# gstoica27/ReLUQP-py

Hardware: AMD Instinct MI355X
Metric: QP solves/sec (batch=4096 random dense QPs n=100 m=300) (higher is better)
Workload: dtype f32; 1 GPU; batch=4096/GPU random dense QPs n=100 m=300 (n_eq=25), feasible rand_qp seeds 0.., eps_abs=0.001, cold start, reference defaults; 4 distinct batches in rotation, every solve without dispatch history (= first solve of a fresh handle); global_batch=4096, parallelism=batch-split x1, no collectives, kernel=resident2, tile=same, low_memory=False, fresh_batches=4, dispatch_history=False, rho_window=5

## Files before the change

reluqp-py_amd/csrc/rqp_resident2.hip:

```cpp
#include <cstdio>
#include <cstdlib>
#include <type_traits>
#include <vector>

#include "rqp_common.h"

typedef float f2 __attribute__((ext_vector_type(2)));
typedef _Float16 h2 __attribute__((ext_vector_type(2)));

__device__ __forceinline__ float fma_mix_lo(h2 k, float v, float acc) {
    asm("v_fma_mix_f32 %0, %1, %2, %0 op_sel_hi:[1,0,0]" : "+v"(acc) : "v"(k), "v"(v));
    return acc;
}
__device__ __forceinline__ float fma_mix_hi(h2 k, float v, float acc) {
    asm("v_fma_mix_f32 %0, %1, %2, %0 op_sel:[1,0,0] op_sel_hi:[1,0,0]" : "+v"(acc) : "v"(k), "v"(v));
    return acc;
}
template <int CTRL>
__device__ __forceinline__ float dpp2(float v) {
    return __builtin_bit_cast(float, __builtin_amdgcn_update_dpp(0, __builtin_bit_cast(int, v), CTRL, 0xF, 0xF, true));
}
__device__ __forceinline__ float swsum32(float a, float b) {
    asm volatile("s_nop 1\n\tv_permlane32_swap_b32 %0, %1" : "+v"(a), "+v"(b));
    return a + b;
}
__device__ __forceinline__ float swsum16(float a, float b) {
    asm volatile("s_nop 1\n\tv_permlane16_swap_b32 %0, %1" : "+v"(a), "+v"(b));
    return a + b;
}
__device__ __forceinline__ float swmax32(float a, float b) {
    asm volatile("s_nop 1\n\tv_permlane32_swap_b32 %0, %1" : "+v"(a), "+v"(b));
    return fmaxf(a, b);
}
__device__ __forceinline__ float swmax16(float a, float b) {
    asm volatile("s_nop 1\n\tv_permlane16_swap_b32 %0, %1" : "+v"(a), "+v"(b));
    return fmaxf(a, b);
}
__device__ __forceinline__ float wave_max(float v) {
    v = fmaxf(v, dpp2<0xB1>(v));
    v = fmaxf(v, dpp2<0x4E>(v));
    v = fmaxf(v, dpp2<0x141>(v));
    v = fmaxf(v, dpp2<0x128>(v));
    float a = v, b = v;
    asm volatile("s_nop 1\n\tv_permlane16_swap_b32 %0, %1" : "+v"(a), "+v"(b));
    v = fmaxf(a, b);
    a = v; b = v;
    asm volatile("s_nop 1\n\tv_permlane32_swap_b32 %0, %1" : "+v"(a), "+v"(b));
    return fmaxf(a, b);
}
__device__ __forceinline__ unsigned wave_or(unsigned v) {
    v |= (unsigned)__builtin_amdgcn_update_dpp(0, (int)v, 0xB1, 0xF, 0xF, true);
    v |= (unsigned)__builtin_amdgcn_update_dpp(0, (int)v, 0x4E, 0xF, 0xF, true);
    v |= (unsigned)__builtin_amdgcn_update_dpp(0, (int)v, 0x141, 0xF, 0xF, true);
    v |= (unsigned)__builtin_amdgcn_update_dpp(0, (int)v, 0x128, 0xF, 0xF, true);
    unsigned a = v, b = v;
    asm volatile("s_nop 1\n\tv_permlane16_swap_b32 %0, %1" : "+v"(a), "+v"(b));
    v = a | b;
    a = v; b = v;
    asm volatile("s_nop 1\n\tv_permlane32_swap_b32 %0, %1" : "+v"(a), "+v"(b));
    return a | b;
}
template <typename T>
__device__ __forceinline__ T tmax2(T a, T b) {
    return (a != a) ? a : ((b != b) ? b : (a > b ? a : b));
}

template <int RB_, int CQ_, int KR_, int KC_>
struct Res2Cfg {
    static constexpr int RB = RB_, CQ = CQ_, KR = KR_, KC = KC_;
    static constexpr int NT = 256, NW = 4, NQ = 2, PL = 32;
    static constexpr int RP = RB / 2, KP = KR / 2;
    static constexpr int CW = NQ * CQ;
    static constexpr int N = NW * CW;
    static constexpr int M = PL * RB;
    static constexpr int SW = 8 * KR + 4;
    static constexpr int ND = NW * SW;
    static constexpr int AE2 = RP * CQ;
    static constexpr int KE2 = KP * KC;
    static constexpr int HR = 4, HP = HR / 2;
    static constexpr int HE2 = HP * CQ;
    static constexpr int HU = HE2 / 2;
    static constexpr int H1 = (CQ + 1) / 2, H2 = (H1 + 1) / 2;
    static constexpr int MATREGS = 2 * (RP * CQ + KP * KC);
    static constexpr int WAVES_PER_SIMD = (MATREGS > 100) ? 2 : ((MATREGS > 30) ? 3 : 4);
    static_assert(RB % 2 == 0 && KR % 2 == 0 && HP == 2 && HU == CQ && PL * HR >= N, "row pairs");
    static_assert(8 * KR >= CW && 8 * KC >= N && M <= 2 * NT && KC == CQ && NQ == 2, "tile shape");
    static constexpr size_t lds_bytes() {
        return (size_t)M * 8 * 4 + ND * 8 + 16 * 8
               + (size_t)M * 4 * 5
               + (size_t)ND * 4 * 6
               + (size_t)NW * M * 4 + 96 * 4
               + (size_t)HU * NT * 16;
    }
};

constexpr int NSEG = 25;
template <class C, bool DIAG, bool KH, bool KD = false>
__global__ void __launch_bounds__(256, C::WAVES_PER_SIMD) k_admm_res2(SolveArgs a, const float* __restrict__ Apack,
                                                      const float* __restrict__ Kpack,
                                                      const float* __restrict__ Hpack, unsigned long long* dbg,
                                                      const float* __restrict__ Kscale) {
    constexpr int RB = C::RB, CQ = C::CQ, KR = C::KR, KC = C::KC, NT = C::NT, NW = C::NW, RP = C::RP, KP = C::KP;
    constexpr int CW = C::CW, M = C::M, ND = C::ND, SW = C::SW, AE2 = C::AE2, KE2 = C::KE2, HU = C::HU, HP = C::HP, HR = C::HR, H1 = C::H1, H2 = C::H2;
    extern __shared__ __attribute__((aligned(16))) unsigned char smem_raw[];
    double* zt64 = (double*)smem_raw;
    double* lam64 = zt64 + M;
    double* z64 = lam64 + M;
    double* inv64 = z64 + M;
    double* x64 = inv64 + M;
    double* redd = x64 + ND;
    float* lT = (float*)(redd + 16);
    float* uT = lT + M;
    float* rv32 = uT + M;
    float* nu = rv32 + M;
    float* cT = nu + M;
    float* xin = cT + M;
    float* xnat = xin + ND;
    float* dxv = xnat + ND;
    float* hx = dxv + ND;
    float* gT = hx + ND;
    float* dvec = gT + ND;
    float* part = dvec + ND;
    float* red = part + NW * M;
    float* Hs = red + 96;
    static_assert(((size_t)M * 8 * 4 + ND * 8 + 16 * 8 + (size_t)M * 4 * 5 + ND * 4 * 6 + NW * M * 4 + 96 * 4) % 16 == 0,
                  "H image must start 16-byte aligned");

    const int n = a.n, m = a.m;
    const int b = a.order ? a.order[blockIdx.x] : (int)blockIdx.x, tid = threadIdx.x;
    const int wave = tid >> 6, lane = tid & 63;
    const int q = lane & 1, pl = lane >> 1, rr = lane >> 3, cc = lane & 7;
    const size_t mat = (a.sA == 0) ? 0 : (size_t)b;
    const float* cg = (const float*)a.c + (size_t)b * m;
    int k0 = 0;
    bool exact = false;
    if (a.cont == 1) {
        if (a.info.status[b] != RQP_STATUS_CONTINUE) {
            if (!(a.warm_starting || a.keep_state)) {
                for (int i = tid; i < n; i += NT) a.x[(size_t)b * n + i] = 0.0;
                for (int i = tid; i < m; i += NT) {
                    a.z[(size_t)b * m + i] = 0.0;
                    a.lam[(size_t)b * m + i] = 0.0;
                }
                if (tid == 0) a.rho_ind[b] = a.rho_ind0;
            }
            return;
        }
        k0 = a.cont_iter[b];
    } else if (a.cont == 2) {
        if (a.gate && *a.gate == 0) return;
        if (a.cstat[b] == 0) return;
        const int ci = a.cont_iter[b];
        if (ci >= 0) {
            k0 = ci;
            exact = true;
        }
    }
    const int wb = a.wbase ? a.wbase[mat] : 0;
    if (a.cstat && a.mode == 0) {
        const int sl = a.rho_ind[b] - wb;
        if (sl < 0 || sl >= a.kwin) {
            if (tid == 0) {
                a.cstat[b] = 1;
                if (!exact) a.cont_iter[b] = -1;
                atomicAdd(a.ncont, 1);
            }
            return;
        }
    }

    f2 ar[RP][CQ];
    {
        const f2* Ap = (const f2*)(Apack + mat * (size_t)AE2 * NT * 2) + tid;
#pragma unroll
        for (int rp = 0; rp < RP; ++rp)
#pragma unroll
            for (int c = 0; c < CQ; ++c) ar[rp][c] = Ap[(size_t)(rp * CQ + c) * NT];
        const float4* Hp = (const float4*)(Hpack + mat * (size_t)HU * NT * 4);
#pragma unroll
        for (int u = 0; u < HU; ++u) ((float4*)Hs)[u * NT + tid] = Hp[u * NT + tid];
    }
    int ri = a.rho_ind[b];
    float* rhoL = red + 64;
    if (tid < 32) rhoL[tid] = (tid < a.nrho) ? (float)a.rhos[tid] : 0.f;
    typedef typename std::conditional<KH, h2, f2>::type kpair_t;
    kpair_t kr[KP][KC];
    float kscale = 1.f;
    auto load_K = [&](int jl) {
        int j = jl - wb;
        j = j < 0 ? 0 : (j >= a.kwin ? a.kwin - 1 : j);
        if constexpr (!KD) {
            int tid_k = tid;
            asm volatile("" : "+v"(tid_k));
            const kpair_t* Kp = (const kpair_t*)Kpack + (mat * a.kwin + j) * (size_t)KE2 * NT + tid_k;
#pragma unroll
            for (int kp = 0; kp < KP; ++kp)
#pragma unroll
                for (int c = 0; c < KC; ++c) kr[kp][c] = Kp[(size_t)(kp * KC + c) * NT];
            if constexpr (KH) kscale = Kscale[mat * a.kwin + j];
        } else {
            int lane_o = lane, wave_o = wave;
            asm volatile("" : "+v"(lane_o), "+v"(wave_o));
            const int rr = lane_o >> 3, cc = lane_o & 7, wave = wave_o;
            const float* Kj = (const float*)a.K + ((a.sK == 0) ? (size_t)0 : (size_t)b * a.sK) + (size_t)j * n * a.ldn;
            typedef float f4u __attribute__((ext_vector_type(4), aligned(4)));
#pragma unroll
            for (int kp = 0; kp < KP; ++kp) {
                const int lr = KR * rr + 2 * kp, r = CW * wave + lr;
                const bool ok0 = lr < CW && r < n, ok1 = lr + 1 < CW && r + 1 < n;
                const float* row0 = Kj + (size_t)(r < n ? r : n - 1) * a.ldn + KC * cc;
                const float* row1 = Kj + (size_t)(r + 1 < n ? r + 1 : n - 1) * a.ldn + KC * cc;
                float t0[KC], t1[KC];
#pragma unroll
                for (int c = 0; c + 4 <= KC; c += 4) {
                    const f4u u0 = *(const f4u*)(row0 + c), u1 = *(const f4u*)(row1 + c);
#pragma unroll
                    for (int e = 0; e < 4; ++e) { t0[c + e] = u0[e]; t1[c + e] = u1[e]; }
                }
#pragma unroll
                for (int c = KC - KC % 4; c < KC; ++c) { t0[c] = row0[c]; t1[c] = row1[c]; }
                const f2 msk = {ok0 ? 1.f : 0.f, ok1 ? 1.f : 0.f};
#pragma unroll
                for (int c = 0; c < KC; ++c) kr[kp][c] = (f2){t0[c], t1[c]} * msk;
            }
        }
    };
    load_K(ri);

    auto set_rho_rows = [&](int j) {
        const float rho = (float)a.rhos[j];
        for (int i = tid; i < M; i += NT) {
            const float rv = rho * ((i < m) ? cg[i] : 1.f);
            rv32[i] = rv;
            inv64[i] = 1.0 / (double)rv;
        }
    };
    for (int i = tid; i < M; i += NT) {
        const bool in = i < m;
        zt64[i] = (exact && in) ? a.ax[(size_t)b * m + i] : 0.0;
        z64[i] = in ? a.z[(size_t)b * m + i] : 0.0;
        lam64[i] = in ? a.lam[(size_t)b * m + i] : 0.0;
        lT[i] = in ? ((const float*)a.l)[(size_t)b * m + i] : 0.f;
        uT[i] = in ? ((const float*)a.u)[(size_t)b * m + i] : 0.f;
        nu[i] = 0.f;
        cT[i] = in ? cg[i] : 1.f;
    }
    set_rho_rows(ri);
    for (int i = tid; i < ND; i += NT) {
        const int col = CW * (i / SW) + (i % SW);
        const bool in = (i % SW) < CW && col < n;
        const double xv = in ? a.x[(size_t)b * n + col] : 0.0;
        x64[i] = xv;
        xin[i] = (float)xv;
        xnat[i] = (i < n) ? (float)a.x[(size_t)b * n + i] : 0.f;
        gT[i] = in ? ((const float*)a.g)[(size_t)b * n + col] : 0.f;
        hx[i] = 0.f;
        dxv[i] = 0.f;
        dvec[i] = 0.f;
    }

    int colw, ncolw;
    {
        const int b5 = (lane >> 5) & 1, b4 = (lane >> 4) & 1;
        const int cbase = H2 * b4 + H1 * b5;
        int nval = b4 ? (H1 - H2) : H2;
        if (b5 && cbase + nval > CQ) nval = CQ - cbase;
        ncolw = ((lane & 0xE) == 0) ? nval : 0;
        colw = SW * wave + CQ * q + cbase;
    }
    __syncthreads();

    auto load_vc = [&](const float* v, float (&vc)[CQ]) __attribute__((always_inline)) {
#pragma unroll
        for (int c = 0; c < CQ; ++c) vc[c] = v[SW * wave + CQ * q + c];
    };
    auto prod_A = [&](const float (&vc)[CQ]) __attribute__((always_inline)) {
        f2 acc[RP];
#pragma unroll
        for (int rp = 0; rp < RP; ++rp) {
            f2 s = {0.f, 0.f};
#pragma unroll
            for (int c = 0; c < CQ; ++c) s = __builtin_elementwise_fma(ar[rp][c], (f2){vc[c], vc[c]}, s);
            s.x += dpp2<0xB1>(s.x);
            s.y += dpp2<0xB1>(s.y);
            acc[rp] = s;
        }
        if (q == 0) {
            f2* dst = (f2*)(part + wave * M + RB * pl);
#pragma unroll
            for (int rp = 0; rp < RP; ++rp) dst[rp] = acc[rp];
        }
    };
    auto prod_At = [&](auto use_a, auto use_h, const float* w, float* out, bool addg) {
        constexpr bool USE_A = decltype(use_a)::value, USE_H = decltype(use_h)::value;
        f2 wr[RP];
        f2 wx[HP];
        if constexpr (USE_A) {
#pragma unroll
            for (int rp = 0; rp < RP; ++rp) wr[rp] = ((const f2*)(w + RB * pl))[rp];
        }
        if constexpr (USE_H) {
            const float4 xv = *(const float4*)(xnat + HR * pl);
            wx[0] = (f2){xv.x, xv.y};
            wx[1] = (f2){xv.z, xv.w};
        }
        auto hload = [&](int c) -> float4 { return ((const float4*)Hs)[c * NT + tid]; };
        auto colsum = [&](int c, const float4& hv) -> float {
            f2 t2 = {0.f, 0.f};
            if constexpr (USE_A) {
#pragma unroll
                for (int rp = 0; rp < RP; ++rp) t2 = __builtin_elementwise_fma(ar[rp][c], wr[rp], t2);
            }
            if constexpr (USE_H) {
                t2 = __builtin_elementwise_fma((f2){hv.x, hv.y}, wx[0], t2);
                t2 = __builtin_elementwise_fma((f2){hv.z, hv.w}, wx[1], t2);
            }
            return t2.x + t2.y;
        };
        float s1[H1];
        auto colsum2 = [&](int c0, int c1, const float4& h0, const float4& h1, float& a0, float& a1) __attribute__((always_inline)) {
            f2 t0 = {0.f, 0.f}, t1 = {0.f, 0.f};
            if constexpr (USE_A) {
#pragma unroll
                for (int rp = 0; rp < RP; ++rp) {
                    t0 = __builtin_elementwise_fma(ar[rp][c0], wr[rp], t0);
                    t1 = __builtin_elementwise_fma(ar[rp][c1], wr[rp], t1);
                }
            }
            if constexpr (USE_H) {
                t0 = __builtin_elementwise_fma((f2){h0.x, h0.y}, wx[0], t0);
                t1 = __builtin_elementwise_fma((f2){h1.x, h1.y}, wx[0], t1);
                t0 = __builtin_elementwise_fma((f2){h0.z, h0.w}, wx[1], t0);
                t1 = __builtin_elementwise_fma((f2){h1.z, h1.w}, wx[1], t1);
            }
            a0 = t0.x + t0.y;
            a1 = t1.x + t1.y;
        };
        float4 hcur = {0.f, 0.f, 0.f, 0.f}, hnext = {0.f, 0.f, 0.f, 0.f};
        if constexpr (USE_H) {
            hcur = hload(0);
            if (H1 < CQ) hnext = hload(H1);
        }
#pragma unroll
        for (int i = 0; i < H1; ++i) {
            const bool pair = (i + H1 < CQ);
            if (pair) {
                float4 hc2 = hcur, hn2 = hnext;
                if constexpr (USE_H) {
                    if (i + 1 < H1) hc2 = hload(i + 1);
                    if (i + 1 + H1 < CQ) hn2 = hload(i + 1 + H1);
                }
                float a0, a1;
                colsum2(i, i + H1, hcur, hnext, a0, a1);
                s1[i] = swsum32(a0, a1);
                hcur = hc2;
                hnext = hn2;
            } else {
                const float a0 = colsum(i, hcur);
                s1[i] = swsum32(a0, a0);
            }
        }
        float gpre[H2];
#pragma unroll
        for (int i = 0; i < H2; ++i) gpre[i] = addg ? gT[colw + i] : 0.f;
        float s2[H2];
#pragma unroll
        for (int i = 0; i < H2; ++i) s2[i] = (i + H2 < H1) ? swsum16(s1[i], s1[i + H2]) : swsum16(s1[i], s1[i]);
#pragma unroll
        for (int i = 0; i < H2; ++i) {
            float v = s2[i];
            v += dpp2<0x4E>(v);
            v += dpp2<0x124>(v);
            v += dpp2<0x128>(v);
            s2[i] = v;
        }
        if (ncolw > 0) {
#pragma unroll
            for (int i = 0; i < H2; ++i)
                if (i < ncolw) out[colw + i] = s2[i] + gpre[i];
        }
    };
    constexpr std::true_type YES{};
    auto prod_At_chk = [&](const float* w, float* outA, float* outH) {
        f2 wr[RP];
        f2 wx[HP];
#pragma unroll
        for (int rp = 0; rp < RP; ++rp) wr[rp] = ((const f2*)(w + RB * pl))[rp];
        {
            const float4 xv = *(const float4*)(xnat + HR * pl);
            wx[0] = (f2){xv.x, xv.y};
            wx[1] = (f2){xv.z, xv.w};
        }
        auto hload = [&](int c) -> float4 { return ((const float4*)Hs)[c * NT + tid]; };
        float sA[H1], sH[H1];
        float4 hcur = hload(0), hnext = {0.f, 0.f, 0.f, 0.f};
        if (H1 < CQ) hnext = hload(H1);
#pragma unroll
        for (int i = 0; i < H1; ++i) {
            const bool pair = (i + H1 < CQ);
            float4 hc2 = hcur, hn2 = hnext;
            if (i + 1 < H1) hc2 = hload(i + 1);
            if (i + 1 + H1 < CQ) hn2 = hload(i + 1 + H1);
            f2 a0 = {0.f, 0.f}, a1 = {0.f, 0.f};
            f2 h0 = __builtin_elementwise_fma((f2){hcur.x, hcur.y}, wx[0], (f2){0.f, 0.f}), h1 = {0.f, 0.f};
            if (pair) h1 = __builtin_elementwise_fma((f2){hnext.x, hnext.y}, wx[0], h1);
#pragma unroll
            for (int rp = 0; rp < RP; ++rp) {
                a0 = __builtin_elementwise_fma(ar[rp][i], wr[rp], a0);
                if (pair) a1 = __builtin_elementwise_fma(ar[rp][i + H1], wr[rp], a1);
            }
            h0 = __builtin_elementwise_fma((f2){hcur.z, hcur.w}, wx[1], h0);
            if (pair) h1 = __builtin_elementwise_fma((f2){hnext.z, hnext.w}, wx[1], h1);
            const float ca0 = a0.x + a0.y, ch0 = h0.x + h0.y;
            sA[i] = pair ? swsum32(ca0, a1.x + a1.y) : swsum32(ca0, ca0);
            sH[i] = pair ? swsum32(ch0, h1.x + h1.y) : swsum32(ch0, ch0);
            hcur = hc2;
            hnext = hn2;
        }
        float tA[H2], tH[H2];
#pragma unroll
        for (int i = 0; i < H2; ++i) {
            tA[i] = (i + H2 < H1) ? swsum16(sA[i], sA[i + H2]) : swsum16(sA[i], sA[i]);
            tH[i] = (i + H2 < H1) ? swsum16(sH[i], sH[i + H2]) : swsum16(sH[i], sH[i]);
        }
#pragma unroll
        for (int i = 0; i < H2; ++i) {
            float va = tA[i], vh = tH[i];
            va += dpp2<0x4E>(va);
            vh += dpp2<0x4E>(vh);
            va += dpp2<0x124>(va);
            vh += dpp2<0x124>(vh);
            va += dpp2<0x128>(va);
            vh += dpp2<0x128>(vh);
            tA[i] = va;
            tH[i] = vh;
        }
        if (ncolw > 0) {
#pragma unroll
            for (int i = 0; i < H2; ++i)
                if (i < ncolw) {
                    outA[colw + i] = tA[i] + 0.f;
                    outH[colw + i] = tH[i] + 0.f;
                }
        }
    };
    auto prod_K = [&](const float* v, float (&s)[KR]) {
        float vc[KC];
#pragma unroll
        for (int c = 0; c < KC; ++c) vc[c] = v[SW * (cc >> 1) + CQ * (cc & 1) + c];
#pragma unroll
        for (int kp = 0; kp < KP; ++kp) {
            f2 t = {0.f, 0.f};
            if constexpr (KH) {
#pragma unroll
                for (int c = 0; c < KC; ++c) {
                    t.x = fma_mix_lo(kr[kp][c], vc[c], t.x);
                    t.y = fma_mix_hi(kr[kp][c], vc[c], t.y);
                }
                t.x *= kscale;
                t.y *= kscale;
            } else {
#pragma unroll
                for (int c = 0; c < KC; ++c) t = __builtin_elementwise_fma(kr[kp][c], (f2){vc[c], vc[c]}, t);
            }
            s[2 * kp] = t.x;
            s[2 * kp + 1] = t.y;
        }
#pragma unroll
        for (int r = 0; r < KR; ++r) s[r] += dpp2<0xB1>(s[r]);
#pragma unroll
        for (int r = 0; r < KR; ++r) s[r] += dpp2<0x4E>(s[r]);
#pragma unroll
        for (int r = 0; r < KR; ++r) s[r] += dpp2<0x141>(s[r]);
    };
    float cv[3] = {0.f, 0.f, 0.f};
    auto row_body = [&](auto nr, bool init, bool do_a, bool do_b, bool chk) __attribute__((always_inline)) {
        constexpr int R = decltype(nr)::value;
        double zt[R], z[R], lmv[R], iv[R];
        float adx[R][NW], lo[R], hi[R], rvf[R];
#pragma unroll
        for (int q = 0; q < R; ++q) {
            const int i = tid + q * NT;
            zt[q] = zt64[i];
            lmv[q] = lam64[i];
            if (do_a) {
                iv[q] = inv64[i];
                lo[q] = lT[i];
                hi[q] = uT[i];
            } else {
                z[q] = z64[i];
            }
            rvf[q] = rv32[i];
            if (init || do_a) {
#pragma unroll
                for (int w = 0; w < NW; ++w) adx[q][w] = part[w * M + i];
            }
        }
        asm volatile("s_waitcnt lgkmcnt(0)" ::: "memory");
#pragma unroll
        for (int q = 0; q < R; ++q) {
            asm volatile("" : "+v"(zt[q]), "+v"(lmv[q]), "+v"(rvf[q]));
            if (do_a) asm volatile("" : "+v"(iv[q]), "+v"(lo[q]), "+v"(hi[q]));
            else asm volatile("" : "+v"(z[q]));
            if (init || do_a) asm volatile("" : "+v"(adx[q][0]), "+v"(adx[q][1]), "+v"(adx[q][2]), "+v"(adx[q][3]));
        }
#pragma unroll
        for (int q = 0; q < R; ++q) {
            const int i = tid + q * NT;
            if (init || do_a) {
                const float ad = ((adx[q][0] + adx[q][1]) + adx[q][2]) + adx[q][3];
                zt[q] = (init ? 0.0 : zt[q]) + (double)ad;
                zt64[i] = zt[q];
            }
            if (do_a) {
                const double v = zt[q] + lmv[q] * iv[q];
                z[q] = v;
                if (v < (double)lo[q]) z[q] = (double)lo[q];
                if (v > (double)hi[q]) z[q] = (double)hi[q];
                z64[i] = z[q];
            }
            if (do_b) {
                const double rv = (double)rvf[q];
                const double pr = zt[q] - z[q];
                const double lh = lmv[q] + rv * pr;
                lam64[i] = lh;
                nu[i] = (float)(lh + rv * pr);
            }
        }
        if (chk) {
            int tid_w = tid;
            asm volatile("" : "+v"(tid_w));
#pragma unroll
            for (int q = 0; q < R; ++q) {
                const int i = tid_w + q * NT;
                const float we = (a.scE && i < m) ? (float)(1.0 / a.scE[mat * m + i]) : 1.f;
                nu[i] = (float)lmv[q];
                cv[0] = tmax2(cv[0], fabsf((float)(zt[q] - z[q])) * we);
                cv[1] = tmax2(cv[1], fabsf((float)zt[q]) * we);
                cv[2] = tmax2(cv[2], fabsf((float)z[q]) * we);
            }
        }
    };
    auto row_pass = [&](bool init, bool do_a, bool do_b, bool chk = false) __attribute__((always_inline)) {
        if constexpr (M > NT) {
            static_assert(M <= 2 * NT, "at most two rows per lane");
            if (tid + NT < M) {
                row_body(std::integral_constant<int, 2>{}, init, do_a, do_b, chk);
                return;
            }
        }
        if (tid < M) row_body(std::integral_constant<int, 1>{}, init, do_a, do_b, chk);
    };

    __builtin_amdgcn_s_waitcnt(0x0F70);
    unsigned long long t_last = 0, t_acc[NSEG] = {};
    bool k_pend = false;
    bool diag_on = true;
    auto stamp = [&](int seg) {
        if constexpr (DIAG) {
            __builtin_amdgcn_sched_barrier(0);
            unsigned long long t;
            asm volatile("s_memtime %0\n\ts_waitcnt lgkmcnt(0)" : "=s"(t)::"memory");
            __builtin_amdgcn_sched_barrier(0);
            if (seg >= 0 && diag_on) t_acc[seg] += t - t_last;
            t_last = t;
        }
    };

    float rho_est = (a.mode == 2) ? (float)a.rho_in : ((a.cont == 1 || exact) ? (float)a.cont_rho[b] : (float)a.rhos[ri]);
    float pri = 0.f, dua = 0.f;
    bool converged = false;
    int iters = k0;
    const float tolT = (float)a.tol;
    const int kmax = (a.mode == 2) ? 0 : a.max_iter;

    if (!exact) {
        float vc0[CQ];
        load_vc(xin, vc0);
        prod_A(vc0);
        __syncthreads();
        row_pass(true, false, kmax > k0);
    } else {
        row_pass(false, false, kmax > k0);
    }

    float scl_p = 0.f, scl_d = 0.f;
    auto res_rows = [&]() {
        cv[0] = cv[1] = cv[2] = 0.f;
        int tid_w = tid;
        asm volatile("" : "+v"(tid_w));
        for (int i = tid_w; i < M; i += NT) {
            const float we = (a.scE && i < m) ? (float)(1.0 / a.scE[mat * m + i]) : 1.f;
            nu[i] = (float)lam64[i];
            cv[0] = tmax2(cv[0], fabsf((float)(zt64[i] - z64[i])) * we);
            cv[1] = tmax2(cv[1], fabsf((float)zt64[i]) * we);
            cv[2] = tmax2(cv[2], fabsf((float)z64[i]) * we);
        }
    };
    int rpar = 0;
    auto residuals = [&](float rho_carry, float& o_pri, float& o_dua) -> float {
        float v[7];
#pragma unroll
        for (int e = 0; e < 3; ++e) v[e] = cv[e];
#pragma unroll
        for (int e = 3; e < 7; ++e) v[e] = 0.f;
        int tid_w = tid;
        asm volatile("" : "+v"(tid_w));
        __syncthreads();
        stamp(10);
        if (tid < ND && (tid % SW) >= CW) {
            dxv[tid] = 0.f;
            hx[tid] = 0.f;
        }
        prod_At_chk(nu, dxv, hx);
        stamp(11);
        __syncthreads();
        stamp(13);
        if (tid < ND) {
            float wd = 1.f;
            if (a.scD) {
                const int col = CW * (tid_w / SW) + (tid_w % SW);
                if ((tid_w % SW) < CW && col < n) wd = (float)(1.0 / (a.scC[mat] * a.scD[mat * n + col]));
            }
            const float t3 = dxv[tid];
            v[3] = fabsf(hx[tid] + t3 + gT[tid]) * wd;
            v[4] = fabsf(hx[tid]) * wd;
            v[5] = fabsf(t3) * wd;
            v[6] = fabsf(gT[tid]) * wd;
        }
        unsigned nanm = 0;
#pragma unroll
        for (int e = 0; e < 7; ++e) nanm |= (__builtin_amdgcn_ballot_w64(v[e] != v[e]) != 0ull) ? (1u << e) : 0u;
        float u0, u1;
        {
            const float r0 = swmax32(v[0], v[4]), r1 = swmax32(v[1], v[5]), r2 = swmax32(v[2], v[6]), r3 = swmax32(v[3], v[3]);
            u0 = swmax16(r0, r2);
            u1 = swmax16(r1, r3);
        }
        u0 = fmaxf(u0, dpp2<0xB1>(u0));
        u1 = fmaxf(u1, dpp2<0xB1>(u1));
        u0 = fmaxf(u0, dpp2<0x4E>(u0));
        u1 = fmaxf(u1, dpp2<0x4E>(u1));
        u0 = fmaxf(u0, dpp2<0x141>(u0));
        u1 = fmaxf(u1, dpp2<0x141>(u1));
        u0 = fmaxf(u0, dpp2<0x128>(u0));
        u1 = fmaxf(u1, dpp2<0x128>(u1));
        float* redp = red + 32 * rpar;
        rpar ^= 1;
        if ((lane & 15) == 0) {
            const int row = lane >> 4;
            *(f2*)(redp + wave * 8 + 2 * row) = (f2){u0, row == 3 ? __builtin_bit_cast(float, nanm) : u1};
        }
        stamp(14);
        __syncthreads();
        stamp(15);
        nanm = 0;
#pragma unroll
        for (int w = 0; w < NW; ++w) nanm |= __builtin_bit_cast(unsigned, redp[w * 8 + 7]);
#pragma unroll
        for (int e = 0; e < 7; ++e) {
            float r = redp[e];
#pragma unroll
            for (int w = 1; w < NW; ++w) r = fmaxf(r, redp[w * 8 + e]);
            v[e] = ((nanm >> e) & 1u) ? __builtin_nanf("") : r;
        }
        stamp(16);
        o_pri = v[0];
        o_dua = v[3];
        scl_p = tmax2(v[1], v[2]);
        scl_d = tmax2(tmax2(v[4], v[5]), v[6]);
        const float num = v[0] / scl_p;
        const float den = v[3] / scl_d;
        float est = rho_carry * sqrtf(num / den);
        if (est < (float)a.rho_min) est = (float)a.rho_min;
        if (est > (float)a.rho_max) est = (float)a.rho_max;
        return est;
    };

    stamp(-1);
    int to_chk = a.check_interval - (k0 % a.check_interval);
    for (int k = k0 + 1; k <= kmax; ++k) {
        __syncthreads();
        stamp(0);
        prod_At(YES, YES, nu, dvec, true);
        stamp(1);
        __syncthreads();
        stamp(2);
        __builtin_amdgcn_s_waitcnt(0x0F70);
        if constexpr (DIAG) {
            if (k_pend) { stamp(20); k_pend = false; }
        }
        {
            float s[KR];
            static_assert(KR == 4 || KR == 2, "vectorised x update");
            const int j = SW * wave + KR * rr;
            double2* xp = (double2*)(x64 + j);
            double2 xold[KR / 2];
#pragma unroll
            for (int hlf = 0; hlf < KR / 2; ++hlf) xold[hlf] = xp[hlf];
            prod_K(dvec, s);
            if (cc == 0) {
#pragma unroll
                for (int hlf = 0; hlf < KR / 2; ++hlf) ((f2*)(dxv + j))[hlf] = (f2){-s[2 * hlf], -s[2 * hlf + 1]};
            }
            __builtin_amdgcn_fence(__ATOMIC_RELEASE, "wavefront");
            __builtin_amdgcn_wave_barrier();
            float vc[CQ];
            load_vc(dxv, vc);
            if (cc == 0) {
                f2* xn2 = (f2*)(xnat + CW * wave + KR * rr);
#pragma unroll
                for (int hlf = 0; hlf < KR / 2; ++hlf) {
                    double2 xa = xold[hlf];
                    const f2 dx = {-s[2 * hlf], -s[2 * hlf + 1]};
                    xa.x += (double)dx.x;
                    xa.y += (double)dx.y;
                    xp[hlf] = xa;
                    const f2 xf = {(float)xa.x, (float)xa.y};
                    ((f2*)(xin + j))[hlf] = xf;
                    if (KR * rr + 2 * hlf + 1 < CW) xn2[hlf] = xf;
                }
            }
            stamp(3);
            prod_A(vc);
        }
        stamp(4);
        __syncthreads();
        stamp(5);
        stamp(6);
        iters = k;
        const bool on_grid = (--to_chk == 0);
        if (on_grid) to_chk = a.check_interval;
        const bool check = (a.mode == 0) && on_grid;
        if (!check) {
            row_pass(false, true, k < kmax);
            stamp(7);
        } else {
            cv[0] = cv[1] = cv[2] = 0.f;
            row_pass(false, true, false, true);
            stamp(8);
            if constexpr (DIAG) t_acc[22] += 1;
            const int ri_before = ri;
            rho_est = residuals(rho_est, pri, dua);
            rho_est = __builtin_bit_cast(float, __builtin_amdgcn_readfirstlane(__builtin_bit_cast(int, rho_est)));
            pri = __builtin_bit_cast(float, __builtin_amdgcn_readfirstlane(__builtin_bit_cast(int, pri)));
            dua = __builtin_bit_cast(float, __builtin_amdgcn_readfirstlane(__builtin_bit_cast(int, dua)));
            if (rho_est > rhoL[ri] * tolT && ri < a.nrho - 1)
                ri += 1;
            else if (rho_est < rhoL[ri] / tolT && ri > 0)
                ri -= 1;
            if (a.info.trace && (k / a.check_interval) <= a.info.trace_cap && tid == 0) {
                double* tr = a.info.trace + ((size_t)b * a.info.trace_cap + (k / a.check_interval - 1)) * 4;
                tr[0] = (double)pri; tr[1] = (double)dua; tr[2] = (double)rho_est; tr[3] = (double)ri_before;
            }
            float tp = (float)a.thr_p, td = (float)a.thr_d;
            if (a.eps_rel > 0) {
                tp += (float)a.eps_rel * __builtin_bit_cast(float, __builtin_amdgcn_readfirstlane(__builtin_bit_cast(int, scl_p)));
                td += (float)a.eps_rel * __builtin_bit_cast(float, __builtin_amdgcn_readfirstlane(__builtin_bit_cast(int, scl_d)));
            }
            stamp(18);
            if (pri < tp && dua < td) {
                converged = true;
                break;
            }
            if (ri != ri_before) {
                if (a.cstat && k < kmax && (ri < wb || ri >= wb + a.kwin)) {
                    int tid_o = tid;
                    asm volatile("" : "+v"(tid_o));
                    for (int i = tid_o; i < n; i += NT) a.x[(size_t)b * n + i] = x64[SW * (i / CW) + i % CW];
                    for (int i = tid_o; i < m; i += NT) {
                        a.z[(size_t)b * m + i] = z64[i];
                        a.lam[(size_t)b * m + i] = lam64[i];
                        a.ax[(size_t)b * m + i] = zt64[i];
                    }
                    if (tid_o == 0) {
                        a.rho_ind[b] = ri;
                        a.cont_iter[b] = k;
                        a.cont_rho[b] = (double)rho_est;
                        a.cstat[b] = 1;
                        atomicAdd(a.ncont, 1);
                    }
                    return;
                }
                if constexpr (DIAG) { t_acc[23] += 1; k_pend = true; }
                if constexpr (!KD) load_K(ri);
                {
                    int tid_o = tid;
                    asm volatile("" : "+v"(tid_o));
                    const float rho = rhoL[ri];
                    for (int i = tid_o; i < M; i += NT) {
                        const float rv = rho * cT[i];
                        rv32[i] = rv;
                        inv64[i] = 1.0 / (double)rv;
                    }
                }
                if constexpr (KD) load_K(ri);
                stamp(19);
            }
            if (k < kmax) row_pass(false, false, true);
            stamp(21);
        }
    }
    if constexpr (DIAG) {
        diag_on = false;
        if (lane == 0)
            for (int e = 0; e < NSEG; ++e) dbg[((size_t)b * 4 + wave) * NSEG + e] = (e == NSEG - 1) ? (unsigned long long)iters : t_acc[e];
    }

    __syncthreads();
    if (a.mode == 1) {
        for (int i = tid; i < n; i += NT) a.x[(size_t)b * n + i] = x64[SW * (i / CW) + i % CW];
        for (int i = tid; i < m; i += NT) {
            a.z[(size_t)b * m + i] = z64[i];
            a.lam[(size_t)b * m + i] = lam64[i];
        }
        return;
    }
    if (!converged) {
        res_rows();
        rho_est = residuals(rho_est, pri, dua);
    }

    double jp = 0.0;
    if (tid < ND) jp = (double)(xin[tid] * (0.5f * hx[tid] + gT[tid]));
    for (int off = 32; off >= 1; off >>= 1) jp += __shfl_xor(jp, off, 64);
    if (lane == 0) redd[wave] = jp;
    __syncthreads();
    const double obj = redd[0] + redd[1] + redd[2] + redd[3];

    if (a.mode == 2) {
        if (tid == 0) {
            if (a.r_pri) a.r_pri[b] = (double)pri;
            if (a.r_dua) a.r_dua[b] = (double)dua;
            if (a.r_rho) a.r_rho[b] = (double)rho_est;
            if (a.r_obj) a.r_obj[b] = obj;
        }
        return;
    }

    if (a.out_x) for (int i = tid; i < n; i += NT) ((float*)a.out_x)[(size_t)b * n + i] = (float)x64[SW * (i / CW) + i % CW];
    if (a.out_z) for (int i = tid; i < m; i += NT) ((float*)a.out_z)[(size_t)b * m + i] = (float)z64[i];
    if (a.out_lam) for (int i = tid; i < m; i += NT) ((float*)a.out_lam)[(size_t)b * m + i] = (float)lam64[i];
    if (tid == 0) {
        if (a.cstat) a.cstat[b] = 0;
        if (a.info.iter) a.info.iter[b] = converged ? iters : a.max_iter;
        if (a.last_iter) a.last_iter[b] = converged ? iters : a.max_iter;
        if (a.info.status) a.info.status[b] = converged ? RQP_STATUS_SOLVED : ((pri != pri || dua != dua) ? RQP_STATUS_NAN : RQP_STATUS_MAX_ITER);
        if (a.info.rho_ind) a.info.rho_ind[b] = ri;
        if (a.info.pri_res) a.info.pri_res[b] = (double)pri;
        if (a.info.dua_res) a.info.dua_res[b] = (double)dua;
        if (a.info.rho_estimate) a.info.rho_estimate[b] = (double)rho_est;
        if (a.info.obj_val) a.info.obj_val[b] = obj;
    }
    if ((a.warm_starting || a.keep_state)) {
        for (int i = tid; i < n; i += NT) a.x[(size_t)b * n + i] = x64[SW * (i / CW) + i % CW];
        for (int i = tid; i < m; i += NT) {
            a.z[(size_t)b * m + i] = z64[i];
            a.lam[(size_t)b * m + i] = lam64[i];
        }
        if (tid == 0) a.rho_ind[b] = ri;
    } else {
        for (int i = tid; i < n; i += NT) a.x[(size_t)b * n + i] = 0.0;
        for (int i = tid; i < m; i += NT) {
            a.z[(size_t)b * m + i] = 0.0;
            a.lam[(size_t)b * m + i] = 0.0;
        }
        if (tid == 0) a.rho_ind[b] = a.rho_ind0;
    }
}

template <class C, bool KH>
__global__ void k_pack_res2(int n, int ldn, int nrho, const float* __restrict__ K, float* __restrict__ Kpack, float* __restrict__ Kscale,
                            const int32_t* __restrict__ only, const int32_t* __restrict__ gate) {
    constexpr int KR = C::KR, KC = C::KC, NT = C::NT, CW = C::CW, KE2 = C::KE2;
    const int mat = blockIdx.y;
    if (gate && *gate == 0) return;
    if (only && !only[mat]) return;
    const int t = threadIdx.x, w = t >> 6, lane = t & 63;
    const int rr = lane >> 3, cc = lane & 7;
    extern __shared__ __attribute__((aligned(16))) float stage[];
    {
        const int j = blockIdx.x;
        const float* Kj = K + ((size_t)mat * nrho + j) * n * ldn;
        for (int i = t; i < n * ldn; i += NT) stage[i] = Kj[i];
        __syncthreads();
        float inv_scale = 1.f;
        if constexpr (KH) {
            __shared__ float smax[NT];
            float mx = 0.f;
            for (int i = t; i < n * ldn; i += NT) mx = fmaxf(mx, fabsf(stage[i]));
            smax[t] = mx;
            __syncthreads();
            for (int off = NT / 2; off >= 1; off >>= 1) {
                if (t < off) smax[t] = fmaxf(smax[t], smax[t + off]);
                __syncthreads();
            }
            int e2 = 0;
            (void)frexpf(fmaxf(smax[0], 1e-30f), &e2);
            const float sc = ldexpf(1.f, e2 - 14);
            inv_scale = ldexpf(1.f, 14 - e2);
            if (t == 0) Kscale[(size_t)mat * nrho + j] = sc;
        }
        float* Kp = Kpack + ((size_t)mat * nrho + j) * KE2 * NT * (KH ? 1 : 2);
        for (int pair = 0; pair < KE2; ++pair) {
            const int lr = KR * rr + 2 * (pair / KC);
            const int r = CW * w + lr, c = KC * cc + pair % KC;
            f2 v;
            v.x = (lr < CW && r < n && c < n) ? stage[r * ldn + c] : 0.f;
            v.y = (lr + 1 < CW && r + 1 < n && c < n) ? stage[(r + 1) * ldn + c] : 0.f;
            if constexpr (KH)
                ((h2*)Kp)[(size_t)pair * NT + t] = (h2){(_Float16)(v.x * inv_scale), (_Float16)(v.y * inv_scale)};
            else
                ((f2*)Kp)[(size_t)pair * NT + t] = v;
        }
    }
}


template <class C>
__global__ void k_pack_res2_ah(int n, int m, int ldn, const float* __restrict__ A, const float* __restrict__ Ht,
                               float* __restrict__ Apack, float* __restrict__ Hpack) {
    constexpr int RB = C::RB, CQ = C::CQ, NT = C::NT, CW = C::CW, AE2 = C::AE2, HU = C::HU, HR = C::HR, RCH = C::M / 4;
    const int mat = blockIdx.y, ch = blockIdx.x, t = threadIdx.x;
    extern __shared__ __attribute__((aligned(16))) float stage[];
    if (ch < 4) {
        if (!A) return;
        const int r0 = RCH * ch;
        const float* Am = A + (size_t)mat * m * ldn + (size_t)r0 * ldn;
        const int avail = (m - r0) * ldn;
        if ((((size_t)Am) & 15) == 0) {
            for (int i = 4 * t; i < RCH * ldn; i += 4 * NT)
                *(float4*)(stage + i) = (i < avail) ? *(const float4*)(Am + i) : (float4){0.f, 0.f, 0.f, 0.f};
        } else {
            for (int i = t; i < RCH * ldn; i += NT) stage[i] = (i < avail) ? Am[i] : 0.f;
        }
        __syncthreads();
        const int l16 = t & 15, w = (t >> 4) & 3, part = t >> 6;
        const int lane = 16 * ch + l16, q = lane & 1, pl = lane >> 1, tk = 64 * w + lane;
        f2* Ap = (f2*)(Apack + (size_t)mat * AE2 * NT * 2);
        for (int pair = part; pair < AE2; pair += 4) {
            const int lr = RB * pl + 2 * (pair / CQ) - r0, c = CW * w + CQ * q + pair % CQ;
            f2 v;
            v.x = (c < n) ? stage[lr * ldn + c] : 0.f;
            v.y = (c < n) ? stage[(lr + 1) * ldn + c] : 0.f;
            Ap[(size_t)pair * NT + tk] = v;
        }
    } else {
        const int w = t >> 6, lane = t & 63, q = lane & 1, pl = lane >> 1;
        const float* Hm = Ht + (size_t)mat * n * ldn;
        if ((((size_t)Hm) & 15) == 0) {
            for (int i = 4 * t; i < n * ldn; i += 4 * NT) *(float4*)(stage + i) = *(const float4*)(Hm + i);
        } else {
            for (int i = t; i < n * ldn; i += NT) stage[i] = Hm[i];
        }
        __syncthreads();
        float4* Hp = (float4*)(Hpack + (size_t)mat * HU * NT * 4);
        for (int c0 = 0; c0 < CQ; ++c0) {
            const int c = CW * w + CQ * q + c0;
            float hv[HR];
            for (int h = 0; h < HR; ++h) {
                const int r = HR * pl + h;
                hv[h] = (r < n && c < n) ? stage[c * ldn + r] : 0.f;
            }
            Hp[(size_t)c0 * NT + t] = (float4){hv[0], hv[1], hv[2], hv[3]};
        }
    }
}

typedef Res2Cfg<10, 13, 4, 13> Cfg2C2;
typedef Res2Cfg<2, 4, 2, 4> Cfg2C4;
typedef Res2Cfg<4, 7, 2, 7> Cfg2M;
typedef Res2Cfg<10, 10, 4, 10> Cfg2N;

static int res2_pick(const rqp_handle* h) {
    if (h->esz != 4 || h->nrho > 32) return -1;
    if (h->n <= Cfg2C4::N && h->m <= Cfg2C4::M) return 0;
    if (h->n <= Cfg2M::N && h->m <= Cfg2M::M) return 1;
    if (h->n <= Cfg2N::N && h->m <= Cfg2N::M) return 3;
    if (h->n <= Cfg2C2::N && h->m <= Cfg2C2::M) return 2;
    return -1;
}

bool rqp_res2_fits(const rqp_handle* h) { return res2_pick(h) >= 0; }

template <class C>
static void pack_elems_t(const rqp_handle* h, size_t* a_elems, size_t* k_elems, size_t* h_elems) {
    *a_elems = (size_t)h->nmat * C::AE2 * C::NT * 2;
    *k_elems = h->k_direct ? 0 : (size_t)h->nmat * h->kwin * C::KE2 * C::NT * (h->dims.tile_dtype == RQP_TILE_F16 ? 1 : 2);
    *h_elems = (size_t)h->nmat * C::HU * C::NT * 4;
}
void rqp_res2_pack_elems(const rqp_handle* h, size_t* a_elems, size_t* k_elems, size_t* h_elems) {
    switch (res2_pick(h)) {
        case 0: pack_elems_t<Cfg2C4>(h, a_elems, k_elems, h_elems); break;
        case 1: pack_elems_t<Cfg2M>(h, a_elems, k_elems, h_elems); break;
        case 3: pack_elems_t<Cfg2N>(h, a_elems, k_elems, h_elems); break;
        default: pack_elems_t<Cfg2C2>(h, a_elems, k_elems, h_elems); break;
    }
}

void rqp_res2_kp_layout(const rqp_handle* h, int* cw, int* kr, int* kc) {
    switch (res2_pick(h)) {
        case 0: *cw = Cfg2C4::CW; *kr = Cfg2C4::KR; *kc = Cfg2C4::KC; break;
        case 1: *cw = Cfg2M::CW; *kr = Cfg2M::KR; *kc = Cfg2M::KC; break;
        case 3: *cw = Cfg2N::CW; *kr = Cfg2N::KR; *kc = Cfg2N::KC; break;
        default: *cw = Cfg2C2::CW; *kr = Cfg2C2::KR; *kc = Cfg2C2::KC; break;
    }
}

template <class C>
static hipError_t pack_t(const rqp_handle* h, const void* A_src, const int32_t* only, const int32_t* gate, hipStream_t s) {
    const size_t stage_ah = (size_t)(C::M / 4 > h->n ? C::M / 4 : h->n) * h->ldn * sizeof(float);
    const size_t stage_k = (size_t)h->n * h->ldn * sizeof(float);
    if (!only)
        k_pack_res2_ah<C><<<dim3(5, h->nmat), C::NT, stage_ah, s>>>(h->n, h->m, h->ldn, (const float*)A_src, (const float*)h->Ht, h->Apack, h->Hpack);
    if (h->dims.tile_dtype == RQP_TILE_F16) {
        k_pack_res2<C, true><<<dim3(h->kwin, h->nmat), C::NT, stage_k, s>>>(h->n, h->ldn, h->kwin, (const float*)h->K, h->Kpack, h->Kscale, only, gate);
    } else {
        if (!h->k_direct && !h->kpack_direct)
            k_pack_res2<C, false><<<dim3(h->kwin, h->nmat), C::NT, stage_k, s>>>(h->n, h->ldn, h->kwin, (const float*)h->K, h->Kpack, nullptr, only, gate);
    }
    return hipGetLastError();
}
hipError_t rqp_launch_pack_res2(const rqp_handle* h, const void* A_src, const int32_t* only, const int32_t* gate, hipStream_t s) {
    switch (res2_pick(h)) {
        case 0: return pack_t<Cfg2C4>(h, A_src, only, gate, s);
        case 1: return pack_t<Cfg2M>(h, A_src, only, gate, s);
        case 3: return pack_t<Cfg2N>(h, A_src, only, gate, s);
        default: return pack_t<Cfg2C2>(h, A_src, only, gate, s);
    }
}

template <class C>
static hipError_t prepare_t(const rqp_handle* h) {
    const size_t lds = C::lds_bytes();
    {
        const size_t stage_ah = (size_t)(C::M / 4 > h->n ? C::M / 4 : h->n) * h->ldn * sizeof(float);
        hipError_t ae = rqp_raise_lds_limit((const void*)k_pack_res2_ah<C>, stage_ah);
        if (ae != hipSuccess) return ae;
    }
    {
        const size_t stage = (size_t)h->n * h->ldn * sizeof(float);
        hipError_t pe = (h->dims.tile_dtype == RQP_TILE_F16)
                            ? rqp_raise_lds_limit((const void*)k_pack_res2<C, true>, (size_t)stage)
                            : rqp_raise_lds_limit((const void*)k_pack_res2<C, false>, (size_t)stage);
        if (pe != hipSuccess) return pe;
    }
    if (h->dims.tile_dtype == RQP_TILE_F16)
        return rqp_raise_lds_limit((const void*)k_admm_res2<C, false, true>, (size_t)lds);
    hipError_t e = rqp_raise_lds_limit((const void*)k_admm_res2<C, false, false>, (size_t)lds);
    if (e != hipSuccess) return e;
    if (h->k_direct) {
        e = rqp_raise_lds_limit((const void*)k_admm_res2<C, false, false, true>, (size_t)lds);
        if (e != hipSuccess) return e;
    }
    if (h->debug & 2) e = rqp_raise_lds_limit((const void*)k_admm_res2<C, true, false>, (size_t)lds);
    if (h->debug & 1) {
        int nb = -1;
        hipError_t oe = hipOccupancyMaxActiveBlocksPerMultiprocessor(&nb, k_admm_res2<C, false, false>, C::NT, lds);
        hipFuncAttributes fa;
        (void)hipFuncGetAttributes(&fa, (const void*)k_admm_res2<C, false, false>);
        fprintf(stderr, "[rqp] k_admm_res2<%d,%d,%d,%d>: blocks/CU=%d (err %d) lds=%zu B regs=%d scratch=%zu B\n", C::RB, C::CQ,
                C::KR, C::KC, nb, (int)oe, lds, fa.numRegs, (size_t)fa.localSizeBytes);
    }
    return e;
}
hipError_t rqp_prepare_res2(const rqp_handle* h) {
    switch (res2_pick(h)) {
        case 0: return prepare_t<Cfg2C4>(h);
        case 1: return prepare_t<Cfg2M>(h);
        case 3: return prepare_t<Cfg2N>(h);
        default: return prepare_t<Cfg2C2>(h);
    }
}

template <class C>
static hipError_t solve_t(const rqp_handle* h, const SolveArgs& a, hipStream_t s) {
    const size_t lds = C::lds_bytes();
    if (h->dims.tile_dtype == RQP_TILE_F16) {
        k_admm_res2<C, false, true><<<h->B, C::NT, lds, s>>>(a, h->Apack, h->Kpack, h->Hpack, nullptr, h->Kscale);
        return hipGetLastError();
    }
    if ((h->debug & 2) && !h->k_direct) {
        const std::vector<double> sums = rqp_diag_run(s, h->B, 4, NSEG, [&](unsigned long long* dbg) {
            k_admm_res2<C, true, false><<<h->B, C::NT, lds, s>>>(a, h->Apack, h->Kpack, h->Hpack, dbg, nullptr);
        });
        if (sums.empty()) return hipErrorOutOfMemory;
        static const char* names[22] = {"B3 wait", "A'nu+Hx", "B1 wait", "Kd+x", "A dx", "B2 wait", "-", "rows",
                                        "rows(a)", "res rows", "R1 wait", "A'lam", "Hx", "R2 wait", "norms+reduce", "R3 wait", "combine",
                                        "R4 wait", "decision", "K issue+rho rows", "K wait", "rows(b)"};
        for (int w = 0; w < 4; ++w) {
            const double* tot = &sums[(size_t)w * NSEG];
            const double its = tot[NSEG - 1], chk = tot[22] > 0 ? tot[22] : 1.0;
            fprintf(stderr, "[rqp diag] wave %d cycles/iteration:", w);
            double sum = 0, csum = 0;
            for (int e = 8; e < 22; ++e) csum += tot[e];
            for (int e = 0; e < 8; ++e) { fprintf(stderr, " %s=%.0f", names[e], tot[e] / its); sum += tot[e] / its; }
            fprintf(stderr, " check=%.0f | total=%.0f\n", csum / its, sum + csum / its);
            fprintf(stderr, "[rqp diag] wave %d cycles/check:", w);
            for (int e = 8; e < 22; ++e) fprintf(stderr, " %s=%.0f", names[e], tot[e] / chk);
            fprintf(stderr, " | total=%.0f ; checks/instance=%.2f moves/instance=%.2f moves/check=%.3f\n", csum / chk, tot[22] / h->B,
                    tot[23] / h->B, tot[23] / chk);
        }
        return hipGetLastError();
    }
    if (h->k_direct)
        k_admm_res2<C, false, false, true><<<h->B, C::NT, lds, s>>>(a, h->Apack, nullptr, h->Hpack, nullptr, nullptr);
    else
        k_admm_res2<C, false, false><<<h->B, C::NT, lds, s>>>(a, h->Apack, h->Kpack, h->Hpack, nullptr, nullptr);
    return hipGetLastError();
}
hipError_t rqp_launch_solve_res2(const rqp_handle* h, const SolveArgs& a, hipStream_t s) {
    switch (res2_pick(h)) {
        case 0: return solve_t<Cfg2C4>(h, a, s);
        case 1: return solve_t<Cfg2M>(h, a, s);
        case 3: return solve_t<Cfg2N>(h, a, s);
        default: return solve_t<Cfg2C2>(h, a, s);
    }
}
```

Before: 1.415 million QP/s.

## Overlap kernel prologue loads with counted vmcnt waits and add fixed-cost diag stamps

Restructures the kernel prologue so that all per-instance vector loads (z, lam, l, u, c, x, g, rhos) are issued into registers first. The H image and the first part of the A tile are issued after them, and counted s_waitcnt vmcnt waits then let the vector LDS initialisation proceed while the matrix loads are still in flight. The rest of the A tile and the K tile are issued before the row setup, and the final wait keeps the K loads outstanding (vmcnt=KE2) instead of draining everything. The goal is to hide global-load latency in the cold-start prologue. In exchange it adds register pressure and relies on the exact count of memory instructions the compiler emits, which is fragile. It also adds diagnostic timestamps for fixed per-instance phases, active only when the diagnostic template is instantiated.

```diff
diff --git a/reluqp-py_amd/csrc/rqp_resident2.hip b/reluqp-py_amd/csrc/rqp_resident2.hip
--- a/reluqp-py_amd/csrc/rqp_resident2.hip
+++ b/reluqp-py_amd/csrc/rqp_resident2.hip
@@ -64,6 +64,8 @@
 __device__ __forceinline__ T tmax2(T a, T b) {
     return (a != a) ? a : ((b != b) ? b : (a > b ? a : b));
 }
+
+constexpr int vmcnt_imm(int cnt) { return 0x0F70 | (cnt & 15) | ((cnt >> 4) << 14); }
 
 template <int RB_, int CQ_, int KR_, int KC_>
 struct Res2Cfg {
@@ -94,7 +96,7 @@
     }
 };
 
-constexpr int NSEG = 25;
+constexpr int NSEG = 32, SEG_ITERS = 24, SEG_FIXED = 25;
 template <class C, bool DIAG, bool KH, bool KD = false>
 __global__ void __launch_bounds__(256, C::WAVES_PER_SIMD) k_admm_res2(SolveArgs a, const float* __restrict__ Apack,
                                                       const float* __restrict__ Kpack,
@@ -132,6 +134,38 @@
     const int q = lane & 1, pl = lane >> 1, rr = lane >> 3, cc = lane & 7;
     const size_t mat = (a.sA == 0) ? 0 : (size_t)b;
     const float* cg = (const float*)a.c + (size_t)b * m;
+    unsigned long long t_last = 0, t_acc[NSEG] = {};
+    bool k_pend = false;
+    bool diag_on = true;
+    auto stamp = [&](int seg) {
+        if constexpr (DIAG) {
+            __builtin_amdgcn_sched_barrier(0);
+            unsigned long long t;
+            asm volatile("s_memtime %0\n\ts_waitcnt lgkmcnt(0)" : "=s"(t)::"memory");
+            __builtin_amdgcn_sched_barrier(0);
+            if (seg >= 0 && diag_on) t_acc[seg] += t - t_last;
+            t_last = t;
+        }
+    };
+    unsigned long long t_fix = 0;
+    auto fstamp = [&](int seg) {
+        if constexpr (DIAG) {
+            __builtin_amdgcn_sched_barrier(0);
+            unsigned long long t;
+            asm volatile("s_memtime %0\n\ts_waitcnt lgkmcnt(0)" : "=s"(t)::"memory");
+            __builtin_amdgcn_sched_barrier(0);
+            if (seg >= 0) t_acc[seg] += t - t_fix;
+            t_fix = t;
+        }
+    };
+    auto dbg_flush = [&](int iters_dbg) {
+        if constexpr (DIAG) {
+            if (lane == 0)
+                for (int e = 0; e < NSEG; ++e)
+                    dbg[((size_t)b * 4 + wave) * NSEG + e] = (e == SEG_ITERS) ? (unsigned long long)iters_dbg : t_acc[e];
+        }
+    };
+    fstamp(-1);
     int k0 = 0;
     bool exact = false;
     if (a.cont == 1) {
@@ -170,19 +204,8 @@
     }
 
     f2 ar[RP][CQ];
-    {
-        const f2* Ap = (const f2*)(Apack + mat * (size_t)AE2 * NT * 2) + tid;
-#pragma unroll
-        for (int rp = 0; rp < RP; ++rp)
-#pragma unroll
-            for (int c = 0; c < CQ; ++c) ar[rp][c] = Ap[(size_t)(rp * CQ + c) * NT];
-        const float4* Hp = (const float4*)(Hpack + mat * (size_t)HU * NT * 4);
-#pragma unroll
-        for (int u = 0; u < HU; ++u) ((float4*)Hs)[u * NT + tid] = Hp[u * NT + tid];
-    }
     int ri = a.rho_ind[b];
     float* rhoL = red + 64;
-    if (tid < 32) rhoL[tid] = (tid < a.nrho) ? (float)a.rhos[tid] : 0.f;
     typedef typename std::conditional<KH, h2, f2>::type kpair_t;
     kpair_t kr[KP][KC];
     float kscale = 1.f;
@@ -225,39 +248,94 @@
             }
         }
     };
+    int tid_g = tid;
+    asm volatile("" : "+v"(tid_g));
+    constexpr int MR = (M + NT - 1) / NT;
+    constexpr int NA1 = (AE2 < 52 - HU) ? AE2 : 52 - HU;
+    static_assert(MR <= 2 && ND <= NT && HU + NA1 <= 63 && KE2 + 1 <= 63, "counted waits of the prologue");
+    double p_ax[MR], p_z[MR], p_lam[MR], p_rho = 0.0, p_x = 0.0, p_xn = 0.0;
+    float p_l[MR], p_u[MR], p_c[MR], p_g = 0.f;
+    const int scol = CW * (tid_g / SW) + (tid_g % SW);
+    const bool sin = tid_g < ND && (tid_g % SW) < CW && scol < n;
+#pragma unroll
+    for (int r = 0; r < MR; ++r) {
+        const int i = tid_g + r * NT;
+        const bool in = i < m;
+        p_ax[r] = p_z[r] = p_lam[r] = 0.0;
+        p_l[r] = p_u[r] = 0.f;
+        p_c[r] = 1.f;
+        if (exact && in) p_ax[r] = a.ax[(size_t)b * m + i];
+        if (in) {
+            p_z[r] = a.z[(size_t)b * m + i];
+            p_lam[r] = a.lam[(size_t)b * m + i];
+            p_l[r] = ((const float*)a.l)[(size_t)b * m + i];
+            p_u[r] = ((const float*)a.u)[(size_t)b * m + i];
+            p_c[r] = cg[i];
+        }
+    }
+    if (sin) {
+        p_x = a.x[(size_t)b * n + scol];
+        p_g = ((const float*)a.g)[(size_t)b * n + scol];
+    }
+    if (tid_g < n) p_xn = a.x[(size_t)b * n + tid_g];
+    if (tid_g < 32 && tid_g < a.nrho) p_rho = a.rhos[tid_g];
+    double p_rhoi = a.rhos[ri];
+    asm volatile("" ::: "memory");
+    fstamp(SEG_FIXED + 0);
+    const f2* Ap = (const f2*)(Apack + mat * (size_t)AE2 * NT * 2) + tid_g;
+    const float4* Hp = (const float4*)(Hpack + mat * (size_t)HU * NT * 4);
+    {
+        float4 hreg[HU];
+#pragma unroll
+        for (int u = 0; u < HU; ++u) hreg[u] = Hp[u * NT + tid];
+#pragma unroll
+        for (int e = 0; e < NA1; ++e) ar[e / CQ][e % CQ] = Ap[(size_t)e * NT];
+#pragma unroll
+        for (int u = 0; u < HU; ++u) ((float4*)Hs)[u * NT + tid] = hreg[u];
+    }
+    asm volatile("" ::: "memory");
+    fstamp(SEG_FIXED + 1);
+
+    __builtin_amdgcn_s_waitcnt(vmcnt_imm(NA1));
+#pragma unroll
+    for (int r = 0; r < MR; ++r) asm volatile("" : "+v"(p_ax[r]), "+v"(p_z[r]), "+v"(p_lam[r]), "+v"(p_l[r]), "+v"(p_u[r]), "+v"(p_c[r]));
+    asm volatile("" : "+v"(p_x), "+v"(p_xn), "+v"(p_g), "+v"(p_rho), "+v"(p_rhoi));
+    if (tid < 32) rhoL[tid] = (tid < a.nrho) ? (float)p_rho : 0.f;
+    {
+        const float rho = (float)p_rhoi;
+#pragma unroll
+        for (int r = 0; r < MR; ++r) {
+            const int i = tid + r * NT;
+            if (i < M) {
+                zt64[i] = p_ax[r];
+                z64[i] = p_z[r];
+                lam64[i] = p_lam[r];
+                lT[i] = p_l[r];
+                uT[i] = p_u[r];
+                nu[i] = 0.f;
+                cT[i] = p_c[r];
+                const float rv = rho * p_c[r];
+                rv32[i] = rv;
+                inv64[i] = 1.0 / (double)rv;
+            }
+        }
+    }
+    if (tid < ND) {
+        x64[tid] = p_x;
+        xin[tid] = (float)p_x;
+        xnat[tid] = (float)p_xn;
+        gT[tid] = p_g;
+        hx[tid] = 0.f;
+        dxv[tid] = 0.f;
+        dvec[tid] = 0.f;
+    }
+    asm volatile("" ::: "memory");
+    fstamp(SEG_FIXED + 2);
+#pragma unroll
+    for (int e = NA1; e < AE2; ++e) ar[e / CQ][e % CQ] = Ap[(size_t)e * NT];
+    asm volatile("" ::: "memory");
     load_K(ri);
-
-    auto set_rho_rows = [&](int j) {
-        const float rho = (float)a.rhos[j];
-        for (int i = tid; i < M; i += NT) {
-            const float rv = rho * ((i < m) ? cg[i] : 1.f);
-            rv32[i] = rv;
-            inv64[i] = 1.0 / (double)rv;
-        }
-    };
-    for (int i = tid; i < M; i += NT) {
-        const bool in = i < m;
-        zt64[i] = (exact && in) ? a.ax[(size_t)b * m + i] : 0.0;
-        z64[i] = in ? a.z[(size_t)b * m + i] : 0.0;
-        lam64[i] = in ? a.lam[(size_t)b * m + i] : 0.0;
-        lT[i] = in ? ((const float*)a.l)[(size_t)b * m + i] : 0.f;
-        uT[i] = in ? ((const float*)a.u)[(size_t)b * m + i] : 0.f;
-        nu[i] = 0.f;
-        cT[i] = in ? cg[i] : 1.f;
-    }
-    set_rho_rows(ri);
-    for (int i = tid; i < ND; i += NT) {
-        const int col = CW * (i / SW) + (i % SW);
-        const bool in = (i % SW) < CW && col < n;
-        const double xv = in ? a.x[(size_t)b * n + col] : 0.0;
-        x64[i] = xv;
-        xin[i] = (float)xv;
-        xnat[i] = (i < n) ? (float)a.x[(size_t)b * n + i] : 0.f;
-        gT[i] = in ? ((const float*)a.g)[(size_t)b * n + col] : 0.f;
-        hx[i] = 0.f;
-        dxv[i] = 0.f;
-        dvec[i] = 0.f;
-    }
+    fstamp(SEG_FIXED + 1);
 
     int colw, ncolw;
     {
@@ -268,6 +346,7 @@
         ncolw = ((lane & 0xE) == 0) ? nval : 0;
         colw = SW * wave + CQ * q + cbase;
     }
+    fstamp(SEG_FIXED + 2);
     __syncthreads();
 
     auto load_vc = [&](const float* v, float (&vc)[CQ]) __attribute__((always_inline)) {
@@ -552,20 +631,8 @@
         if (tid < M) row_body(std::integral_constant<int, 1>{}, init, do_a, do_b, chk);
     };
 
-    __builtin_amdgcn_s_waitcnt(0x0F70);
-    unsigned long long t_last = 0, t_acc[NSEG] = {};
-    bool k_pend = false;
-    bool diag_on = true;
-    auto stamp = [&](int seg) {
-        if constexpr (DIAG) {
-            __builtin_amdgcn_sched_barrier(0);
-            unsigned long long t;
-            asm volatile("s_memtime %0\n\ts_waitcnt lgkmcnt(0)" : "=s"(t)::"memory");
-            __builtin_amdgcn_sched_barrier(0);
-            if (seg >= 0 && diag_on) t_acc[seg] += t - t_last;
-            t_last = t;
-        }
-    };
+    __builtin_amdgcn_s_waitcnt(KD ? 0x0F70 : vmcnt_imm(KE2));
+    fstamp(SEG_FIXED + 3);
 
     float rho_est = (a.mode == 2) ? (float)a.rho_in : ((a.cont == 1 || exact) ? (float)a.cont_rho[b] : (float)a.rhos[ri]);
     float pri = 0.f, dua = 0.f;
@@ -677,6 +744,7 @@
         return est;
     };
 
+    fstamp(SEG_FIXED + 4);
     stamp(-1);
     int to_chk = a.check_interval - (k0 % a.check_interval);
     for (int k = k0 + 1; k <= kmax; ++k) {
@@ -801,11 +869,8 @@
             stamp(21);
         }
     }
-    if constexpr (DIAG) {
-        diag_on = false;
-        if (lane == 0)
-            for (int e = 0; e < NSEG; ++e) dbg[((size_t)b * 4 + wave) * NSEG + e] = (e == NSEG - 1) ? (unsigned long long)iters : t_acc[e];
-    }
+    diag_on = false;
+    fstamp(-1);
 
     __syncthreads();
     if (a.mode == 1) {
@@ -814,6 +879,7 @@
             a.z[(size_t)b * m + i] = z64[i];
             a.lam[(size_t)b * m + i] = lam64[i];
         }
+        dbg_flush(iters);
         return;
     }
     if (!converged) {
@@ -827,6 +893,7 @@
     if (lane == 0) redd[wave] = jp;
     __syncthreads();
     const double obj = redd[0] + redd[1] + redd[2] + redd[3];
+    fstamp(SEG_FIXED + 5);
 
     if (a.mode == 2) {
         if (tid == 0) {
@@ -835,6 +902,7 @@
             if (a.r_rho) a.r_rho[b] = (double)rho_est;
             if (a.r_obj) a.r_obj[b] = obj;
         }
+        dbg_flush(iters);
         return;
     }
 
@@ -867,6 +935,9 @@
         }
         if (tid == 0) a.rho_ind[b] = a.rho_ind0;
     }
+    if constexpr (DIAG) __builtin_amdgcn_s_waitcnt(0x0F70);
+    fstamp(SEG_FIXED + 6);
+    dbg_flush(iters);
 }
 
 template <class C, bool KH>
@@ -1090,7 +1161,7 @@
                                         "R4 wait", "decision", "K issue+rho rows", "K wait", "rows(b)"};
         for (int w = 0; w < 4; ++w) {
             const double* tot = &sums[(size_t)w * NSEG];
-            const double its = tot[NSEG - 1], chk = tot[22] > 0 ? tot[22] : 1.0;
+            const double its = tot[SEG_ITERS], chk = tot[22] > 0 ? tot[22] : 1.0;
             fprintf(stderr, "[rqp diag] wave %d cycles/iteration:", w);
             double sum = 0, csum = 0;
             for (int e = 8; e < 22; ++e) csum += tot[e];
@@ -1100,6 +1171,12 @@
             for (int e = 8; e < 22; ++e) fprintf(stderr, " %s=%.0f", names[e], tot[e] / chk);
             fprintf(stderr, " | total=%.0f ; checks/instance=%.2f moves/instance=%.2f moves/check=%.3f\n", csum / chk, tot[22] / h->B,
                     tot[23] / h->B, tot[23] / chk);
+            static const char* fixed[NSEG - SEG_FIXED] = {"launch..loads", "matrix issue+H->LDS", "vectors+rho rows", "A wait", "A x+rows",
+                                                          "exit..objective", "stores"};
+            fprintf(stderr, "[rqp diag] wave %d cycles/instance:", w);
+            double fsum = 0;
+            for (int e = SEG_FIXED; e < NSEG; ++e) { fprintf(stderr, " %s=%.0f", fixed[e - SEG_FIXED], tot[e] / h->B); fsum += tot[e] / h->B; }
+            fprintf(stderr, " | total=%.0f\n", fsum);
         }
         return hipGetLastError();
     }
```

Measured after the change: 1.432 million QP/s, median of 6. 1.01x the previous value.
